# Video-Object-Detection/TSCD

Hardware: NVIDIA B200
Metric: clip-frames/sec of TSCD aggregation stage (higher is better)
Workload: dtype f16

## Files before the change

tscd_b200/aggregate.py:

```python
from typing import Dict, Optional

import torch

import os

SINGLE_PASS_MAX_LOGIT = float(os.environ.get("TSCD_ATTN_MAX_LOGIT", "25.0"))

from . import ops

FUSED_QKV = True


class MCAWeights:

    def __init__(self, sd: Dict[str, torch.Tensor], prefix: str, dtype=torch.float16, device="cuda"):
        def w(name):
            return sd[prefix + name].detach().to(device=device, dtype=dtype).contiguous()

        def b(name):
            return sd[prefix + name].detach().to(device=device, dtype=torch.float32).contiguous()

        self.qkv_cls = torch.cat([w("mca.q_cls_local.weight"), w("mca.kv_cls.weight")], 0).contiguous()
        self.qkv_reg = torch.cat([w("mca.q_reg_local.weight"), w("mca.kv_reg.weight")], 0).contiguous()
        self.lin_w, self.lin_b = w("mca.linear.weight"), b("mca.linear.bias")
        self.has_reg = (prefix + "mca.linear_reg.weight") in sd
        if self.has_reg:
            self.linreg_w, self.linreg_b = w("mca.linear_reg.weight"), b("mca.linear_reg.bias")
            self.obj_w, self.obj_b = w("linear_obj.weight"), b("linear_obj.bias")
        self.out_w, self.out_b = w("linear.weight"), b("linear.bias")


def make_layout(sel_count: torch.Tensor, B: int, F: int, L: int, row_cap: int, loc_cap: int, nk_pitch: int,
                dtype=torch.float16, row_off: Optional[torch.Tensor] = None) -> ops.AttnLayoutT:
    if row_off is None:
        cnt = sel_count.view(B, F).to(torch.int32)
        row_off = torch.zeros(B * F + 1, dtype=torch.int32, device=sel_count.device)
        row_off[1:] = torch.cumsum(cnt.reshape(-1), 0)
    lrow_off = torch.empty(B * L + 1, dtype=torch.int32, device=sel_count.device)
    assert sel_count.dtype == torch.int32 and sel_count.is_contiguous()
    ops.call("tscd_local_offsets", ops.L.LocalOffsetsArgs, B=B, F=F, L=L, sel_count=sel_count, lrow_off=lrow_off)
    return ops.AttnLayoutT(B, F, L, row_off, lrow_off, row_cap, loc_cap, nk_pitch, dtype)


def mca_forward(lay: ops.AttnLayoutT, w: MCAWeights, bank_cls, bank_reg, bank_score, n_rows_dev, n_loc_dev,
                need_reg=True, sim_thresh=0.75, conf_sim_thresh=0.99, debug=None, cls_out=(True, True), obj_out=(True, True),
                tag="mca"):
    dev, dt = bank_cls.device, lay.dtype
    tmp_c = torch.empty(lay.loc_cap, 512, dtype=dt, device=dev)
    tmp_r = torch.empty(lay.loc_cap, 512, dtype=dt, device=dev)
    qkv_c = qkv_r = None
    if FUSED_QKV:
        bufs = ops.qkv_project_fused(lay, bank_cls, bank_reg, w.qkv_cls, w.qkv_reg, bank_score, n_rows_dev,
                                     xori_cls=tmp_c[:, 256:], xori_reg=tmp_r[:, 256:], tag=tag)
    else:
        qkv_c, _ = ops.linear(bank_cls, w.qkv_cls, m_dev=n_rows_dev)
        qkv_r, _ = ops.linear(bank_reg, w.qkv_reg, m_dev=n_rows_dev)
        bufs = ops.attn_prep(lay, qkv_c, qkv_r, bank_score, xori_cls=tmp_c[:, 256:], xori_reg=tmp_r[:, 256:])
    stats = torch.empty(lay.loc_cap, 16, dtype=torch.float32, device=dev)
    ops.attn_pv(lay, bufs, tmp_c[:, :256], tmp_r[:, :256], stats, need_reg=need_reg, tag=tag, max_logit=SINGLE_PASS_MAX_LOGIT)
    cat_c = torch.empty(lay.loc_cap, 768, dtype=dt, device=dev)
    ops.linear(tmp_c, w.lin_w, w.lin_b, m_dev=n_loc_dev, out16=cat_c[:, 256:], want16=False, tag=tag + ".mca_linear")
    w_keep = torch.empty(lay.loc_cap, lay.nk_pitch, dtype=dt, device=dev) if need_reg else None
    ops.attn_round2(lay, bufs, bufs["vt_cls"], stats, cat_c[:, :256], use_obj_mask=False, sim_thresh=sim_thresh,
                    conf_sim_thresh=conf_sim_thresh, w_out=w_keep, tag=tag + ".cls")
    trans_cls16, trans_cls32 = ops.linear(cat_c, w.out_w, w.out_b, m_dev=n_loc_dev, want16=cls_out[0], want32=cls_out[1],
                                          tag=tag + ".linear")
    trans_obj16 = trans_obj32 = None
    cat_r = None
    if need_reg:
        cat_r = torch.empty(lay.loc_cap, 768, dtype=dt, device=dev)
        ops.linear(tmp_r, w.linreg_w, w.linreg_b, m_dev=n_loc_dev, out16=cat_r[:, 256:], want16=False, tag=tag + ".mca_linear_reg")
        ops.attn_round2(lay, bufs, bufs["vt_reg"], stats, cat_r[:, :256], use_obj_mask=True, sim_thresh=sim_thresh,
                        conf_sim_thresh=conf_sim_thresh, w_in=w_keep, tag=tag + ".obj")
        trans_obj16, trans_obj32 = ops.linear(cat_r, w.obj_w, w.obj_b, m_dev=n_loc_dev, want16=obj_out[0], want32=obj_out[1],
                                              tag=tag + ".linear_obj")
    if debug is not None:
        debug.update(qkv_c=qkv_c, qkv_r=qkv_r, bufs=bufs, tmp_c=tmp_c, tmp_r=tmp_r, stats=stats, cat_c=cat_c, cat_r=cat_r)
    return (trans_cls16, trans_cls32), (trans_obj16, trans_obj32)


class MSAWeights:

    def __init__(self, sd: Dict[str, torch.Tensor], prefix: str, dtype=torch.float16, device="cuda"):
        w = lambda n: sd[prefix + n].detach().to(device=device, dtype=dtype).contiguous()
        b = lambda n: sd[prefix + n].detach().to(device=device, dtype=torch.float32).contiguous()
        self.qkv_cls, self.qkv_reg = w("msa.qkv_cls.weight"), w("msa.qkv_reg.weight")
        self.l1_w, self.l1_b = w("linear1.weight"), b("linear1.bias")
        self.l2_w, self.l2_b = w("linear2.weight"), b("linear2.bias")


def msa_forward(lay: ops.AttnLayoutT, w: MSAWeights, bank_cls, bank_reg, bank_score, n_rows_dev,
                sim_thresh=0.75, conf_sim_thresh=0.99):
    assert lay.self_attn and lay.L == lay.F
    dev, dt, cap = bank_cls.device, lay.dtype, lay.row_cap
    qkv_c, _ = ops.linear(bank_cls, w.qkv_cls, m_dev=n_rows_dev, tag="msa.qkv_cls")
    qkv_r, _ = ops.linear(bank_reg, w.qkv_reg, m_dev=n_rows_dev, tag="msa.qkv_reg")
    tmp_c = torch.empty(cap, 512, dtype=dt, device=dev)
    tmp_r = torch.empty(cap, 512, dtype=dt, device=dev)
    bufs = ops.attn_prep(lay, qkv_c, qkv_r, bank_score, xori_cls=tmp_c[:, 256:], xori_reg=tmp_r[:, 256:])
    stats = torch.empty(cap, 16, dtype=torch.float32, device=dev)
    ops.attn_pv(lay, bufs, tmp_c[:, :256], tmp_r[:, :256], stats, need_reg=False, tag="msa", max_logit=SINGLE_PASS_MAX_LOGIT)
    cat = torch.empty(cap, 1024, dtype=dt, device=dev)
    ops.linear(tmp_c, w.l1_w, w.l1_b, m_dev=n_rows_dev, out16=cat[:, 512:], want16=False, tag="msa.linear1")
    tct = torch.empty(lay.B * 512, lay.nk_pitch, dtype=dt, device=dev)
    ops.call("tscd_transpose_clip", ops.L.TransposeArgs, lay=lay.to_c(), width=512, x=cat[:, 512:], ld_x=cat.stride(0), xt=tct)
    for half in range(2):
# ... 6 lines not shown
```

tscd_b200/csrc/attn.cu:

```cuda
#include <cuda.h>

#include "common.cuh"
#include "tc.cuh"

namespace tscd {

int make_tmap_kmajor(CUtensorMap* m, const void* ptr, int is_bf16, int64_t rows, int64_t K, int64_t ld, int box_rows);

constexpr int kAttnThreads = 160;
constexpr float kLog2e = 1.4426950408889634f;

template <typename T>
__device__ __forceinline__ float2 ld2(const T* p);
template <> __device__ __forceinline__ float2 ld2<__half>(const __half* p) { return __half22float2(*reinterpret_cast<const __half2*>(p)); }
template <> __device__ __forceinline__ float2 ld2<__nv_bfloat16>(const __nv_bfloat16* p) {
    return __bfloat1622float2(*reinterpret_cast<const __nv_bfloat162*>(p));
}
template <typename T>
__device__ __forceinline__ void st2(T* p, float a, float b);
template <> __device__ __forceinline__ void st2<__half>(__half* p, float a, float b) { *reinterpret_cast<__half2*>(p) = __floats2half2_rn(a, b); }
template <> __device__ __forceinline__ void st2<__nv_bfloat16>(__nv_bfloat16* p, float a, float b) {
    *reinterpret_cast<__nv_bfloat162*>(p) = __floats2bfloat162_rn(a, b);
}

// ... 966 lines not shown
        tmem_dealloc<512>(tmem);
    }
}

static bool layout_ok(const tscd_attn_layout& l) {
    return l.B > 0 && l.F > 0 && l.L > 0 && l.L <= l.F && l.row_cap > 0 && l.nk_pitch > 0 && (l.nk_pitch % 128) == 0 &&
           l.row_off && l.lrow_off && (l.dtype == TSCD_F16 || l.dtype == TSCD_BF16);
}

}

extern "C" int tscd_attn_prep(const tscd_attn_prep_args* a, void* stream) {
    using namespace tscd;
    if (!a || !layout_ok(a->lay)) return TSCD_ERR_INVALID_ARG;
    cudaStream_t st = reinterpret_cast<cudaStream_t>(stream);
    dim3 grid(a->lay.nk_pitch / 64, a->lay.B);
    const size_t smem = 2 * 64 * kPrepRowPitch * 2;
    if (a->lay.dtype == TSCD_F16) {
        if (cudaFuncSetAttribute(attn_prep_kernel<__half>, cudaFuncAttributeMaxDynamicSharedMemorySize, (int)smem) != cudaSuccess) return TSCD_ERR_CUDA;
        attn_prep_kernel<__half><<<grid, kPrepThreads, smem, st>>>(*a);
    } else {
        if (cudaFuncSetAttribute(attn_prep_kernel<__nv_bfloat16>, cudaFuncAttributeMaxDynamicSharedMemorySize, (int)smem) != cudaSuccess) return TSCD_ERR_CUDA;
        attn_prep_kernel<__nv_bfloat16><<<grid, kPrepThreads, smem, st>>>(*a);
    }
    TSCD_CUDA_CHECK_LAUNCH();
    return TSCD_OK;
}

extern "C" int tscd_transpose_clip(const tscd_transpose_args* a, void* stream) {
    using namespace tscd;
    if (!a || !layout_ok(a->lay) || a->width <= 0 || (a->width % 64) != 0) return TSCD_ERR_INVALID_ARG;
    dim3 grid(a->lay.nk_pitch / 64, a->width / 64, a->lay.B);
    cudaStream_t st = reinterpret_cast<cudaStream_t>(stream);
    if (a->lay.dtype == TSCD_F16) transpose_clip_kernel<__half><<<grid, 256, 0, st>>>(*a);
    else transpose_clip_kernel<__nv_bfloat16><<<grid, 256, 0, st>>>(*a);
    TSCD_CUDA_CHECK_LAUNCH();
    return TSCD_OK;
}

extern "C" int tscd_attn_pv(const tscd_attn_pv_args* a, void* stream) {
    using namespace tscd;
    if (!a || !layout_ok(a->lay)) return TSCD_ERR_INVALID_ARG;
    const tscd_attn_layout& l = a->lay;
    const int bf = l.dtype == TSCD_BF16;
    PvTmaps tm;
    int rc = 0;
    rc |= make_tmap_kmajor(&tm.qc, a->qn_cls, bf, l.row_cap, 256, 256, 128);
    rc |= make_tmap_kmajor(&tm.kc, a->kn_cls, bf, l.row_cap, 256, 256, 128);
    rc |= make_tmap_kmajor(&tm.qr, a->qn_reg, bf, l.row_cap, 256, 256, 128);
    rc |= make_tmap_kmajor(&tm.kr, a->kn_reg, bf, l.row_cap, 256, 256, 128);
    rc |= make_tmap_kmajor(&tm.k64c, a->kn_cls, bf, l.row_cap, 256, 256, 64);
    rc |= make_tmap_kmajor(&tm.k64r, a->kn_reg, bf, l.row_cap, 256, 256, 64);
    rc |= make_tmap_kmajor(&tm.vtc, a->vt_cls, bf, (int64_t)l.B * 256, l.nk_pitch, l.nk_pitch, 64);
    rc |= make_tmap_kmajor(&tm.vtr, a->vt_reg, bf, (int64_t)l.B * 256, l.nk_pitch, l.nk_pitch, 64);
    if (rc) return TSCD_ERR_CUDA;
    const size_t smem = 65536 + kPvStages * 32768 + 65536 + sizeof(PvBars);
    dim3 grid((l.nk_pitch + 127) / 128, l.B);
    cudaStream_t st = reinterpret_cast<cudaStream_t>(stream);
    if (bf) {
        if (cudaFuncSetAttribute(attn_pv_kernel<true>, cudaFuncAttributeMaxDynamicSharedMemorySize, (int)smem) != cudaSuccess) return TSCD_ERR_CUDA;
        attn_pv_kernel<true><<<grid, kPvThreads, smem, st>>>(tm, *a);
    } else {
        if (cudaFuncSetAttribute(attn_pv_kernel<false>, cudaFuncAttributeMaxDynamicSharedMemorySize, (int)smem) != cudaSuccess) return TSCD_ERR_CUDA;
        attn_pv_kernel<false><<<grid, kPvThreads, smem, st>>>(tm, *a);
    }
    TSCD_CUDA_CHECK_LAUNCH();
    return TSCD_OK;
}

extern "C" int tscd_attn_round2(const tscd_attn_round2_args* a, void* stream) {
    using namespace tscd;
    if (!a || !layout_ok(a->lay)) return TSCD_ERR_INVALID_ARG;
    if (a->w_in && !a->use_obj_mask) return TSCD_ERR_INVALID_ARG;
    const tscd_attn_layout& l = a->lay;
    const int bf = l.dtype == TSCD_BF16;
    R2Tmaps tm;
    int rc = 0;
    rc |= make_tmap_kmajor(&tm.q128c, a->qn_cls, bf, l.row_cap, 256, 256, 128);
    rc |= make_tmap_kmajor(&tm.q128r, a->qn_reg, bf, l.row_cap, 256, 256, 128);
    rc |= make_tmap_kmajor(&tm.k64c, a->kn_cls, bf, l.row_cap, 256, 256, 64);
    rc |= make_tmap_kmajor(&tm.k64r, a->kn_reg, bf, l.row_cap, 256, 256, 64);
    rc |= make_tmap_kmajor(&tm.vn128c, a->vn_cls, bf, l.row_cap, 256, 256, 128);
    rc |= make_tmap_kmajor(&tm.vn128r, a->vn_reg, bf, l.row_cap, 256, 256, 128);
    rc |= make_tmap_kmajor(&tm.vn64c, a->vn_cls, bf, l.row_cap, 256, 256, 64);
    rc |= make_tmap_kmajor(&tm.vn64r, a->vn_reg, bf, l.row_cap, 256, 256, 64);
    rc |= make_tmap_kmajor(&tm.vt, a->vt, bf, (int64_t)l.B * 256, l.nk_pitch, l.nk_pitch, 64);
    if (rc) return TSCD_ERR_CUDA;
    const size_t smem = kR2SmemBytes + sizeof(R2Bars);
    dim3 grid((l.nk_pitch + 127) / 128, l.B);
    cudaStream_t st = reinterpret_cast<cudaStream_t>(stream);
    if (bf) {
        if (cudaFuncSetAttribute(attn_round2_kernel<true>, cudaFuncAttributeMaxDynamicSharedMemorySize, (int)smem) != cudaSuccess) return TSCD_ERR_CUDA;
        attn_round2_kernel<true><<<grid, kR2Threads, smem, st>>>(tm, *a);
    } else {
        if (cudaFuncSetAttribute(attn_round2_kernel<false>, cudaFuncAttributeMaxDynamicSharedMemorySize, (int)smem) != cudaSuccess) return TSCD_ERR_CUDA;
        attn_round2_kernel<false><<<grid, kR2Threads, smem, st>>>(tm, *a);
    }
    TSCD_CUDA_CHECK_LAUNCH();
    return TSCD_OK;
}

#ifdef TSCD_R2_PROF
extern "C" int tscd_debug_r2_waits(unsigned long long* out, int reset) {
    if (reset) {
        unsigned long long z[64] = {};
        return cudaMemcpyToSymbol(tscd::g_r2_wait, z, sizeof(z)) == cudaSuccess && cudaMemcpyToSymbol(tscd::g_pv_wait, z, sizeof(z)) == cudaSuccess ? 0 : -1;
    }
// ... 16 lines not shown
```

tscd_b200/csrc/gemm.cu:

```cuda
#include <cuda.h>

#include "common.cuh"
#include "tc.cuh"

namespace tscd {

constexpr int kGemmBM = 128;
constexpr int kGemmBK = 64;
constexpr int kGemmStages = 3;
constexpr int kGemmThreads = 320;
constexpr int kGemmThreadsFused = 576;
__host__ __device__ constexpr int gemm_epi_warps(int epi) { return epi ? 16 : 8; }

struct GemmParams {
    int M, N, K;
    const int* m_dev;
    const float* bias;
    void* out16;
    float* out32;
    int ld16, ld32;
    int is_bf16;
    const int32_t* row_meta;
    const int32_t* row_off;
    const int32_t* lrow_off;
    int F, L, self_attn, nk_pitch;
    const float* key_score;
    float scale;
    void *qn, *kn, *vn, *vt, *xori;
    int ld_xori;
};

#ifdef TSCD_R2_PROF
__device__ unsigned long long g_gemm_wait[8];
template <int EPI>
__device__ __forceinline__ void gemm_wait_prof(uint64_t* bar, uint32_t parity, int tag, int slot) {
    const long long t0 = clock64();
    tc::mbar_wait(bar, parity, tag);
    if (EPI == 1 && blockIdx.x == 0 && (threadIdx.x & 31) == 0 && threadIdx.x < 96) atomicAdd(&g_gemm_wait[slot], (unsigned long long)(clock64() - t0));
}
#define GEMM_WAIT(bar, parity, tag, slot) gemm_wait_prof<EPI>(bar, parity, tag, slot)
#else
#define GEMM_WAIT(bar, parity, tag, slot) mbar_wait(bar, parity, tag)
#endif

constexpr int kAccStages = 2;

template <int BN, bool BF16, int EPI = 0>
__global__ void __launch_bounds__(EPI ? kGemmThreadsFused : kGemmThreads) gemm_tn_kernel(const __grid_constant__ CUtensorMap tmap_a,
                                                                const __grid_constant__ CUtensorMap tmap_w,
                                                                const GemmParams p) {
    using namespace tc;
    constexpr int STAGES = BN == 256 ? 4 : 3;
    int M = p.M;
    if (p.m_dev) M = min(M, __ldg(p.m_dev));
    const int tiles_n = (p.N + BN - 1) / BN;
    const int tiles_m = (M + kGemmBM - 1) / kGemmBM;
    const int num_tiles = tiles_m * tiles_n;
    if ((int)blockIdx.x >= num_tiles) return;
#ifdef TSCD_R2_PROF
    const long long tk0 = clock64();
#endif

    extern __shared__ __align__(1024) unsigned char smem_raw[];
    unsigned char* smem = smem_raw;
    constexpr int kABytes = kGemmBM * kGemmBK * 2;
    constexpr int kWBytes = BN * kGemmBK * 2;
    unsigned char* sA = smem;
    unsigned char* sW = smem + STAGES * kABytes;
    unsigned char* sStage = sW + STAGES * kWBytes;
    uint64_t* full_bar = reinterpret_cast<uint64_t*>(sStage + gemm_epi_warps(EPI) * 2048);
    uint64_t* empty_bar = full_bar + STAGES;
    uint64_t* tmem_full_bar = empty_bar + STAGES;
    uint64_t* tmem_empty_bar = tmem_full_bar + kAccStages;
    uint32_t& tmem_base_smem = *reinterpret_cast<uint32_t*>(tmem_empty_bar + kAccStages);
    if ((smem_u32(smem) & 1023u) != 0) __trap();

    const int warp = threadIdx.x >> 5;
    const int lane = threadIdx.x & 31;
    const int num_kb = (p.K + kGemmBK - 1) / kGemmBK;
    const bool w_resident = num_kb == STAGES;
    auto tile_origin = [&](int t, int& m0, int& n0) {
        if (w_resident) { m0 = (t % tiles_m) * kGemmBM; n0 = (t / tiles_m) * BN; }
        else { m0 = (t / tiles_n) * kGemmBM; n0 = (t % tiles_n) * BN; }
    };

    if (warp == 0 && lane == 0) {
        tma_prefetch_desc(&tmap_a);
        tma_prefetch_desc(&tmap_w);
        for (int s = 0; s < STAGES; ++s) { mbar_init(&full_bar[s], 1); mbar_init(&empty_bar[s], 1); }
        for (int s = 0; s < kAccStages; ++s) { mbar_init(&tmem_full_bar[s], 1); mbar_init(&tmem_empty_bar[s], gemm_epi_warps(EPI)); }
        fence_barrier_init();
    }
    if (warp == 1) tmem_alloc<kAccStages * BN>(&tmem_base_smem);
    tc_fence_before();
    __syncthreads();
    tc_fence_after();
    const uint32_t tmem_base = tmem_base_smem;

    if (warp == 0) {
        if (lane == 0) {
            uint32_t it = 0;
            int n_prev = -1;
            for (int t = blockIdx.x; t < num_tiles; t += gridDim.x) {
                int m0, n0;
                tile_origin(t, m0, n0);
                const bool load_w = !(w_resident && n0 == n_prev);
                for (int kb = 0; kb < num_kb; ++kb, ++it) {
                    const int s = it % STAGES;
                    const uint32_t ph = (it / STAGES) & 1;
                    GEMM_WAIT(&empty_bar[s], ph ^ 1, 100 + s, 0);
                    mbar_expect_tx(&full_bar[s], load_w ? kABytes + kWBytes : kABytes);
                    tma_load_2d(sA + s * kABytes, &tmap_a, &full_bar[s], kb * kGemmBK, m0);
                    if (load_w) tma_load_2d(sW + s * kWBytes, &tmap_w, &full_bar[s], kb * kGemmBK, n0);
                }
                n_prev = n0;
            }
        }
    } else if (warp == 1) {
        {
            const uint32_t idesc = make_idesc_f16(BF16, kGemmBM, BN);
            uint32_t it = 0, ti = 0;
            for (int t = blockIdx.x; t < num_tiles; t += gridDim.x, ++ti) {
                const int acc = ti % kAccStages;
                const uint32_t aph = (ti / kAccStages) & 1;
                GEMM_WAIT(&tmem_empty_bar[acc], aph ^ 1, 130 + acc, 1);
                tc_fence_after();
                const uint32_t d = tmem_base + (uint32_t)(acc * BN);
                for (int kb = 0; kb < num_kb; ++kb, ++it) {
                    const int s = it % STAGES;
                    const uint32_t ph = (it / STAGES) & 1;
                    GEMM_WAIT(&full_bar[s], ph, 110 + s, 2);
                    tc_fence_after();
                    const uint64_t adesc = make_smem_desc_sw128(smem_u32(sA + s * kABytes));
                    const uint64_t bdesc = make_smem_desc_sw128(smem_u32(sW + s * kWBytes));
                    if (elect_one()) {
#pragma unroll
                        for (int k = 0; k < kGemmBK / 16; ++k) {
                            umma_f16(d, adesc + (uint64_t)(k * 2), bdesc + (uint64_t)(k * 2), idesc, (kb | k) ? 1u : 0u);
                        }
                        umma_commit(&empty_bar[s]);
                    }
                    __syncwarp();
                }
                if (elect_one()) umma_commit(&tmem_full_bar[acc]);
                __syncwarp();
            }
        }
    } else {
        const int q = warp & 3;
        const int half = (warp - 2) >> 2;
        constexpr int kChunks = BN / 64;
        unsigned char* stg = sStage + (warp - 2) * 2048;
        const bool al16 = p.out16 && (p.ld16 % 8) == 0 && (reinterpret_cast<uintptr_t>(p.out16) & 15) == 0;
        const bool al32 = p.out32 && (p.ld32 % 4) == 0 && (reinterpret_cast<uintptr_t>(p.out32) & 15) == 0;
        uint32_t ti = 0;
        for (int t = blockIdx.x; t < num_tiles; t += gridDim.x, ++ti) {
            int m0, n0;
            tile_origin(t, m0, n0);
            const int acc = ti % kAccStages;
            const uint32_t aph = (ti / kAccStages) & 1;
            const int row_base = m0 + q * 32;
            const int row = row_base + lane;
            const bool row_ok = row < M;
            int meta = -1, lb = 0;
            bool is_query = false;
            if constexpr (EPI == 1) {
                meta = row_ok ? __ldg(p.row_meta + row) : -1;
                if (meta >= 0) {
                    const int cb0 = meta >> 16;
                    const int s0 = __ldg(p.row_off + cb0 * p.F);
                    const int n_loc = (p.self_attn ? __ldg(p.row_off + (cb0 + 1) * p.F) : __ldg(p.row_off + cb0 * p.F + p.L)) - s0;
                    is_query = (meta & 0xffff) < n_loc;
                    lb = __ldg(p.lrow_off + cb0 * p.L);
                }
            }
            GEMM_WAIT(&tmem_full_bar[acc], aph, 120 + acc, 3);
            tc_fence_after();
            const uint32_t tsrc = tmem_base + ((uint32_t)(q * 32) << 16) + (uint32_t)(acc * BN + half * (BN / 2));
            if constexpr (EPI == 1) {
                static_assert(BN == 256 || EPI == 0, "the fused epilogue works on 256-column tiles");
                const int kind = n0 >> 8;
                const bool valid = meta >= 0;
                const int cb = valid ? (meta >> 16) : 0, kr = meta & 0xffff;
                auto pk2h = [](float a, float b) -> uint32_t {
                    if (BF16) { __nv_bfloat162 h = __floats2bfloat162_rn(a, b); return *reinterpret_cast<uint32_t*>(&h); }
                    __half2 h = __floats2half2_rn(a, b);
                    return *reinterpret_cast<uint32_t*>(&h);
                };
                {
                    const int head = (warp - 2) >> 2;
                    const uint32_t tsrc_h = tmem_base + ((uint32_t)(q * 32) << 16) + (uint32_t)(acc * BN + head * 64);
                    uint32_t r0[32], r1[32];
                    tmem_ld_32x32(tsrc_h, r0);
                    tmem_ld_32x32(tsrc_h + 32u, r1);
                    tmem_ld_wait();
                    float ss = 0.f;
#pragma unroll
                    for (int j = 0; j < 32; ++j) {
                        ss = fmaf(__uint_as_float(r0[j]), __uint_as_float(r0[j]), ss);
                        ss = fmaf(__uint_as_float(r1[j]), __uint_as_float(r1[j]), ss);
                    }
                    auto staged_store = [&](const uint32_t (&w16)[16], uint16_t* base, int64_t dest, int ld, int col) {
                        __syncwarp();
#pragma unroll
                        for (int j = 0; j < 4; ++j)
                            *reinterpret_cast<uint4*>(stg + lane * 64 + ((j ^ ((lane >> 1) & 3)) << 4)) =
                                make_uint4(w16[4 * j], w16[4 * j + 1], w16[4 * j + 2], w16[4 * j + 3]);
                        __syncwarp();
#pragma unroll
                        for (int k = 0; k < 4; ++k) {
                            const int rr = 8 * k + (lane >> 2), ch = lane & 3;
                            const uint4 val = *reinterpret_cast<const uint4*>(stg + rr * 64 + ((ch ^ ((rr >> 1) & 3)) << 4));
                            const long long d = __shfl_sync(0xffffffffu, (long long)dest, rr);
                            if (d >= 0) *reinterpret_cast<uint4*>(base + d * ld + col + ch * 8) = val;
                        }
                    };
                    float sc = valid ? 1.f / sqrtf(ss) : 0.f;
                    if (kind == 1 && valid) sc *= p.key_score ? p.scale * __ldg(p.key_score + row) : p.scale;
                    uint16_t* nbase = reinterpret_cast<uint16_t*>(kind == 0 ? p.qn : (kind == 1 ? p.kn : p.vn));
                    const int64_t ndest = (valid && (kind != 0 || is_query)) ? (int64_t)row : -1;
                    uint32_t w16[16];
#pragma unroll
                    for (int j = 0; j < 16; ++j) w16[j] = pk2h(__uint_as_float(r0[2 * j]) * sc, __uint_as_float(r0[2 * j + 1]) * sc);
                    staged_store(w16, nbase, ndest, 256, head * 64);
#pragma unroll
                    for (int j = 0; j < 16; ++j) w16[j] = pk2h(__uint_as_float(r1[2 * j]) * sc, __uint_as_float(r1[2 * j + 1]) * sc);
                    staged_store(w16, nbase, ndest, 256, head * 64 + 32);
                    if (kind == 2) {
                        if (p.xori) {
                            const int64_t xdest = (valid && is_query) ? (int64_t)(lb + kr) : -1;
#pragma unroll
                            for (int j = 0; j < 16; ++j) w16[j] = pk2h(__uint_as_float(r0[2 * j]), __uint_as_float(r0[2 * j + 1]));
                            staged_store(w16, reinterpret_cast<uint16_t*>(p.xori), xdest, p.ld_xori, head * 64);
#pragma unroll
                            for (int j = 0; j < 16; ++j) w16[j] = pk2h(__uint_as_float(r1[2 * j]), __uint_as_float(r1[2 * j + 1]));
                            staged_store(w16, reinterpret_cast<uint16_t*>(p.xori), xdest, p.ld_xori, head * 64 + 32);
                        }
                        if (valid) {
                            uint16_t* vt = reinterpret_cast<uint16_t*>(p.vt) + ((int64_t)cb * 256 + head * 64) * p.nk_pitch + kr;
#pragma unroll
                            for (int j = 0; j < 32; ++j) {
                                vt[(int64_t)j * p.nk_pitch] = (uint16_t)(pk2h(__uint_as_float(r0[j]), 0.f) & 0xffffu);
                                vt[(int64_t)(32 + j) * p.nk_pitch] = (uint16_t)(pk2h(__uint_as_float(r1[j]), 0.f) & 0xffffu);
                            }
                        }
                    }
                    __syncwarp();
                }
                tc_fence_before();
                __syncwarp();
                if (lane == 0) mbar_arrive(&tmem_empty_bar[acc]);
                continue;
            }
            uint32_t rbuf[2][32];
            tmem_ld_32x32(tsrc, rbuf[0]);
            tmem_ld_wait();
#pragma unroll
            for (int c = 0; c < kChunks; ++c) {
                if (c + 1 < kChunks) tmem_ld_32x32(tsrc + (uint32_t)((c + 1) * 32), rbuf[(c + 1) & 1]);
                const uint32_t* r = rbuf[c & 1];
                const int col0 = n0 + half * (BN / 2) + c * 32;
                if (col0 < p.N) {
                    float v[32];
                    if (p.bias) {
#pragma unroll
                        for (int j = 0; j < 32; ++j) v[j] = __uint_as_float(r[j]) + ((col0 + j < p.N) ? __ldg(p.bias + col0 + j) : 0.f);
                    } else {
#pragma unroll
                        for (int j = 0; j < 32; ++j) v[j] = __uint_as_float(r[j]);
                    }
                    const bool full = (col0 + 32 <= p.N);
                    if (p.out16) {
                        uint32_t pk[16];
#pragma unroll
                        for (int j = 0; j < 16; ++j) {
                            if (BF16) {
                                __nv_bfloat162 h = __floats2bfloat162_rn(v[2 * j], v[2 * j + 1]);
                                pk[j] = *reinterpret_cast<uint32_t*>(&h);
                            } else {
                                __half2 h = __floats2half2_rn(v[2 * j], v[2 * j + 1]);
                                pk[j] = *reinterpret_cast<uint32_t*>(&h);
                            }
                        }
                        uint16_t* obase = reinterpret_cast<uint16_t*>(p.out16);
                        __syncwarp();
#pragma unroll
                        for (int j = 0; j < 4; ++j)
                            *reinterpret_cast<uint4*>(stg + lane * 64 + ((j ^ ((lane >> 1) & 3)) << 4)) =
                                make_uint4(pk[4 * j], pk[4 * j + 1], pk[4 * j + 2], pk[4 * j + 3]);
                        __syncwarp();
                        if (full && al16) {
// ... 38 lines not shown
                    }
                }
                if (c + 1 < kChunks) tmem_ld_wait();
            }
            tc_fence_before();
            __syncwarp();
            if (lane == 0) mbar_arrive(&tmem_empty_bar[acc]);
        }
    }
#ifdef TSCD_R2_PROF
    if (EPI == 1 && blockIdx.x == 0 && (threadIdx.x & 31) == 0 && threadIdx.x < 96) atomicAdd(&g_gemm_wait[4 + warp], (unsigned long long)(clock64() - tk0));
#endif
    tc_fence_before();
    __syncthreads();
    if (warp == 1) {
        tc_fence_after();
        tmem_dealloc<kAccStages * BN>(tmem_base);
    }
}

typedef CUresult (*PFN_encodeTiled)(CUtensorMap*, CUtensorMapDataType, cuuint32_t, void*, const cuuint64_t*,
                                    const cuuint64_t*, const cuuint32_t*, const cuuint32_t*, CUtensorMapInterleave,
                                    CUtensorMapSwizzle, CUtensorMapL2promotion, CUtensorMapFloatOOBfill);

static PFN_encodeTiled get_encode() {
    static PFN_encodeTiled fn = nullptr;
    if (!fn) {
        void* p = nullptr;
        cudaDriverEntryPointQueryResult q;
        if (cudaGetDriverEntryPoint("cuTensorMapEncodeTiled", &p, cudaEnableDefault, &q) != cudaSuccess) return nullptr;
        if (q != cudaDriverEntryPointSuccess) return nullptr;
        fn = reinterpret_cast<PFN_encodeTiled>(p);
    }
    return fn;
}

int make_tmap_kmajor(CUtensorMap* m, const void* ptr, int is_bf16, int64_t rows, int64_t K, int64_t ld, int box_rows) {
    PFN_encodeTiled enc = get_encode();
    if (!enc) return TSCD_ERR_CUDA;
    if ((ld * 2) % 16 != 0 || (reinterpret_cast<uintptr_t>(ptr) & 15) != 0) return TSCD_ERR_INVALID_ARG;
    cuuint64_t dims[2] = {(cuuint64_t)K, (cuuint64_t)rows};
    cuuint64_t strides[1] = {(cuuint64_t)(ld * 2)};
    cuuint32_t box[2] = {(cuuint32_t)kGemmBK, (cuuint32_t)box_rows};
    cuuint32_t estr[2] = {1, 1};
    CUresult r = enc(m, is_bf16 ? CU_TENSOR_MAP_DATA_TYPE_BFLOAT16 : CU_TENSOR_MAP_DATA_TYPE_FLOAT16, 2,
                     const_cast<void*>(ptr), dims, strides, box, estr, CU_TENSOR_MAP_INTERLEAVE_NONE,
                     CU_TENSOR_MAP_SWIZZLE_128B, CU_TENSOR_MAP_L2_PROMOTION_L2_256B, CU_TENSOR_MAP_FLOAT_OOB_FILL_NONE);
    return r == CUDA_SUCCESS ? TSCD_OK : TSCD_ERR_CUDA;
}

template <int BN, bool BF16, int EPI = 0>
static int launch_gemm(const CUtensorMap& ta, const CUtensorMap& tw, const GemmParams& p, cudaStream_t st) {
    constexpr int STAGES = BN == 256 ? 4 : 3;
    constexpr size_t smem = (size_t)STAGES * (kGemmBM * kGemmBK * 2 + BN * kGemmBK * 2) + gemm_epi_warps(EPI) * 2048 + 128;
    static bool attr_set[64] = {};
    static int num_sms_dev[64] = {};
    int dev = 0;
    if (cudaGetDevice(&dev) != cudaSuccess || dev < 0 || dev >= 64) return TSCD_ERR_CUDA;
    if (!attr_set[dev]) {
        if (cudaFuncSetAttribute(gemm_tn_kernel<BN, BF16, EPI>, cudaFuncAttributeMaxDynamicSharedMemorySize, (int)smem) != cudaSuccess)
            return TSCD_ERR_CUDA;
        if (cudaDeviceGetAttribute(&num_sms_dev[dev], cudaDevAttrMultiProcessorCount, dev) != cudaSuccess) return TSCD_ERR_CUDA;
        attr_set[dev] = true;
    }
    const int num_sms = num_sms_dev[dev];
    const int tiles = ((p.N + BN - 1) / BN) * ((p.M + kGemmBM - 1) / kGemmBM);
    const int ctas_per_sm = BN == 256 ? 1 : 2;
    const int grid = tiles < ctas_per_sm * num_sms ? tiles : ctas_per_sm * num_sms;
    gemm_tn_kernel<BN, BF16, EPI><<<grid, EPI ? kGemmThreadsFused : kGemmThreads, smem, st>>>(ta, tw, p);
    return cudaGetLastError() == cudaSuccess ? TSCD_OK : TSCD_ERR_CUDA;
}

}

extern "C" int tscd_linear(const tscd_linear_args* a, void* stream) {
    using namespace tscd;
    if (!a || a->M <= 0 || a->N <= 0 || a->K <= 0 || !a->x || !a->w) return TSCD_ERR_INVALID_ARG;
    if (a->dtype != TSCD_F16 && a->dtype != TSCD_BF16) return TSCD_ERR_UNSUPPORTED;
    if (!a->out16 && !a->out32) return TSCD_ERR_INVALID_ARG;
    const int is_bf16 = a->dtype == TSCD_BF16;
    const int BN = a->N <= 64 ? 64 : ((a->N % 256) == 0 && a->K >= 256 ? 256 : 128);
    CUtensorMap ta, tw;
    int rc = make_tmap_kmajor(&ta, a->x, is_bf16, a->M, a->K, a->ldx, kGemmBM);
    if (rc != TSCD_OK) return rc;
    rc = make_tmap_kmajor(&tw, a->w, is_bf16, a->N, a->K, a->ldw, BN);
    if (rc != TSCD_OK) return rc;
    GemmParams p = {};
    p.M = a->M; p.N = a->N; p.K = a->K;
    p.m_dev = a->m_dev; p.bias = a->bias;
    p.out16 = a->out16; p.out32 = a->out32;
    p.ld16 = a->ld16; p.ld32 = a->ld32;
    p.is_bf16 = is_bf16;
    cudaStream_t st = reinterpret_cast<cudaStream_t>(stream);
    if (is_bf16) return BN == 64 ? launch_gemm<64, true>(ta, tw, p, st) : (BN == 128 ? launch_gemm<128, true>(ta, tw, p, st) : launch_gemm<256, true>(ta, tw, p, st));
    return BN == 64 ? launch_gemm<64, false>(ta, tw, p, st) : (BN == 128 ? launch_gemm<128, false>(ta, tw, p, st) : launch_gemm<256, false>(ta, tw, p, st));
}

extern "C" int tscd_qkv_project(const tscd_qkv_project_args* a, void* stream) {
    using namespace tscd;
    if (!a || a->rows <= 0 || !a->x || !a->w || !a->row_meta || !a->qn || !a->kn || !a->vn || !a->vt) return TSCD_ERR_INVALID_ARG;
    const tscd_attn_layout& l = a->lay;
    if (l.dtype != TSCD_F16 && l.dtype != TSCD_BF16) return TSCD_ERR_UNSUPPORTED;
    if (l.B <= 0 || l.F <= 0 || l.L <= 0 || l.L > l.F || !l.row_off || !l.lrow_off || (l.nk_pitch % 128) != 0 || l.nk_pitch > 65536) return TSCD_ERR_INVALID_ARG;
    const int is_bf16 = l.dtype == TSCD_BF16;
    CUtensorMap ta, tw;
    int rc = make_tmap_kmajor(&ta, a->x, is_bf16, a->rows, 256, a->ldx, kGemmBM);
    if (rc != TSCD_OK) return rc;
    rc = make_tmap_kmajor(&tw, a->w, is_bf16, 768, 256, 256, 256);
    if (rc != TSCD_OK) return rc;
    GemmParams p = {};
    p.M = a->rows; p.N = 768; p.K = 256;
    p.m_dev = a->m_dev;
    p.is_bf16 = is_bf16;
    p.row_meta = a->row_meta; p.row_off = l.row_off; p.lrow_off = l.lrow_off;
    p.F = l.F; p.L = l.L; p.self_attn = l.self_attn; p.nk_pitch = l.nk_pitch;
    p.key_score = a->key_score; p.scale = a->scale;
    p.qn = a->qn; p.kn = a->kn; p.vn = a->vn; p.vt = a->vt; p.xori = a->xori; p.ld_xori = a->ld_xori;
    cudaStream_t st = reinterpret_cast<cudaStream_t>(stream);
    return is_bf16 ? launch_gemm<256, true, 1>(ta, tw, p, st) : launch_gemm<256, false, 1>(ta, tw, p, st);
}

#ifdef TSCD_R2_PROF
extern "C" int tscd_debug_gemm_waits(unsigned long long* out, int reset) {
    if (reset) {
        unsigned long long z[8] = {};
        return cudaMemcpyToSymbol(tscd::g_gemm_wait, z, sizeof(z)) == cudaSuccess ? 0 : -1;
    }
    return cudaMemcpyFromSymbol(out, tscd::g_gemm_wait, sizeof(unsigned long long) * 8) == cudaSuccess ? 0 : -1;
}
#endif
```

tscd_b200/ops.py:

```python
import ctypes as C
from dataclasses import dataclass
from typing import List, Optional, Sequence

import torch

from . import _lib as L

_DT = {torch.float32: L.TSCD_F32, torch.float16: L.TSCD_F16, torch.bfloat16: L.TSCD_BF16}


def _stream():
    return C.c_void_p(torch.cuda.current_stream().cuda_stream)


def _p(t: Optional[torch.Tensor]):
    return C.c_void_p(0 if t is None else t.data_ptr())


@dataclass
class AnchorSpec:
    hw: Sequence[Sequence[int]]
    strides: Sequence[int] = (8, 16, 32)

    @property
# ... 345 lines not shown
    if bias is not None:
        assert bias.dtype == torch.float32 and bias.is_contiguous()
    if L.profile is not None:
        L.profile.setdefault("linear", []).append((M, N, K, m_dev, tag, out16 is not None, out32 is not None))
    with L.timed("tscd_linear", tag):
        L.check(L.lib().tscd_linear(C.byref(a), _stream()), "tscd_linear")
    return out16, out32


@dataclass
class AttnLayoutT:
    B: int
    F: int
    L: int
    row_off: torch.Tensor
    lrow_off: torch.Tensor
    row_cap: int
    loc_cap: int
    nk_pitch: int
    dtype: torch.dtype
    self_attn: bool = False

    def to_c(self) -> L.AttnLayout:
        a = L.AttnLayout()
        a.B, a.F, a.L, a.self_attn, a.dtype = self.B, self.F, self.L, int(self.self_attn), _DT[self.dtype]
        a.row_cap, a.nk_pitch = self.row_cap, self.nk_pitch
        a.row_off, a.lrow_off = _p(self.row_off), _p(self.lrow_off)
        return a


def attn_prep(lay: AttnLayoutT, qkv_cls, qkv_reg, key_score, xori_cls=None, xori_reg=None, scale=25.0, bufs=None):
    dev, dt = qkv_cls.device, lay.dtype
    if bufs is None:
        bufs = {}
        for n in ("qn_cls", "kn_cls", "vn_cls", "qn_reg", "kn_reg", "vn_reg"):
            bufs[n] = torch.empty(lay.row_cap, 256, dtype=dt, device=dev)
        for n in ("vt_cls", "vt_reg"):
            bufs[n] = torch.empty(lay.B * 256, lay.nk_pitch, dtype=dt, device=dev)
        bufs["row_frame"] = torch.empty(lay.row_cap, dtype=torch.int32, device=dev)
    a = L.AttnPrepArgs()
    a.lay, a.scale = lay.to_c(), scale
    assert qkv_cls.stride(1) == 1 and qkv_cls.stride(0) == qkv_reg.stride(0)
    a.qkv_cls, a.qkv_reg, a.ld_qkv, a.key_score = _p(qkv_cls), _p(qkv_reg), qkv_cls.stride(0), _p(key_score)
    for n in ("qn_cls", "kn_cls", "vn_cls", "qn_reg", "kn_reg", "vn_reg", "vt_cls", "vt_reg", "row_frame"):
        setattr(a, n, _p(bufs[n]))
    a.xori_cls, a.xori_reg = _p(xori_cls), _p(xori_reg)
    a.ld_xori = 0 if xori_cls is None else xori_cls.stride(0)
    with L.timed("tscd_attn_prep"):
        L.check(L.lib().tscd_attn_prep(C.byref(a), _stream()), "tscd_attn_prep")
    return bufs


def qkv_project_fused(lay: AttnLayoutT, bank_cls, bank_reg, w_cls, w_reg, key_score, n_rows_dev, xori_cls=None, xori_reg=None,
                      scale=25.0, tag=None):
    dev, dt = bank_cls.device, lay.dtype
    bufs = {}
    for n in ("qn_cls", "kn_cls", "vn_cls", "qn_reg", "kn_reg", "vn_reg"):
        bufs[n] = torch.empty(lay.row_cap, 256, dtype=dt, device=dev)
    for n in ("vt_cls", "vt_reg"):
        bufs[n] = torch.empty(lay.B * 256, lay.nk_pitch, dtype=dt, device=dev)
    bufs["row_frame"] = torch.empty(lay.row_cap, dtype=torch.int32, device=dev)
    bufs["row_meta"] = torch.empty(lay.row_cap, dtype=torch.int32, device=dev)
    call("tscd_attn_rowmeta", L.AttnRowmetaArgs, lay=lay.to_c(), row_frame=bufs["row_frame"], row_meta=bufs["row_meta"],
         vt_cls=bufs["vt_cls"], vt_reg=bufs["vt_reg"])
    for br, bank, w, ks, xo in (("cls", bank_cls, w_cls, key_score, xori_cls), ("reg", bank_reg, w_reg, None, xori_reg)):
        assert bank.shape[0] >= lay.row_cap and bank.stride(1) == 1 and w.shape == (768, 256) and w.is_contiguous()
        call("tscd_qkv_project", L.QkvProjectArgs, tag=None if tag is None else f"{tag}.{br}", lay=lay.to_c(), rows=lay.row_cap, m_dev=n_rows_dev, x=bank, ldx=bank.stride(0),
             w=w, row_meta=bufs["row_meta"], key_score=ks, scale=scale, qn=bufs["qn_" + br], kn=bufs["kn_" + br],
             vn=bufs["vn_" + br], vt=bufs["vt_" + br], xori=xo, ld_xori=0 if xo is None else xo.stride(0))
    return bufs


def attn_pv(lay: AttnLayoutT, bufs, x_cls, x_reg, stats, need_reg=True, tag=None, max_logit: float = 0.0):
    a = L.AttnPvArgs()
    a.max_logit = max_logit
    a.lay = lay.to_c()
    for n in ("qn_cls", "kn_cls", "qn_reg", "kn_reg", "vt_cls", "vt_reg", "row_frame"):
        setattr(a, n, _p(bufs[n]))
    a.need_reg = int(need_reg)
    a.x_cls, a.x_reg, a.ld_x, a.stats = _p(x_cls), _p(x_reg), x_cls.stride(0), _p(stats)
    with L.timed("tscd_attn_pv", tag):
        L.check(L.lib().tscd_attn_pv(C.byref(a), _stream()), "tscd_attn_pv")


def attn_round2(lay: AttnLayoutT, bufs, vt, stats, out, use_obj_mask, sim_thresh=0.75, conf_sim_thresh=0.99, w_out=None, w_in=None,
                tag=None):
    a = L.AttnRound2Args()
    a.lay = lay.to_c()
    for n in ("qn_cls", "kn_cls", "qn_reg", "kn_reg", "vn_cls", "vn_reg", "row_frame"):
        setattr(a, n, _p(bufs[n]))
    a.vt, a.stats, a.use_obj_mask = _p(vt), _p(stats), int(use_obj_mask)
    a.sim_thresh, a.conf_sim_thresh = sim_thresh, conf_sim_thresh
    a.out, a.ld_out = _p(out), out.stride(0)
    a.w_out, a.w_in = _p(w_out), _p(w_in)
    for t in (w_out, w_in):
        assert t is None or (t.dtype == lay.dtype and t.stride(0) == lay.nk_pitch and t.stride(1) == 1)
    with L.timed("tscd_attn_round2", tag):
        L.check(L.lib().tscd_attn_round2(C.byref(a), _stream()), "tscd_attn_round2")


def call(name: str, struct_cls, tag=None, **kw):
    a = struct_cls()
    for k, v in kw.items():
        if isinstance(v, C.Structure):
            pass
        elif isinstance(v, torch.Tensor) or v is None:
            v = _p(v)
        elif isinstance(v, torch.dtype):
            v = _DT[v]
        setattr(a, k, v)
    missing = {f[0] for f in struct_cls._fields_} - set(kw)
    assert not missing, f"{name}: missing {missing}"
    with L.timed(name, tag):
        L.check(getattr(L.lib(), name)(C.byref(a), _stream()), name)


def frame_scatter(store, frame_slots: torch.Tensor, sel: dict, status: torch.Tensor, slot_error: Optional[torch.Tensor] = None):
    a = L.FrameScatterArgs()
    a.store = store.to_c()
    a.num_frames = frame_slots.numel()
    a.frame_slots, a.status, a.slot_error = _p(frame_slots), _p(status), _p(slot_error)
    for k in ("sel_count", "row_off", "sel_idx", "sel_rows", "bank_cls", "bank_reg", "bank_edge", "bank_score"):
        setattr(a, k, _p(sel[k]))
    with L.timed("tscd_frame_scatter"):
        L.check(L.lib().tscd_frame_scatter(C.byref(a), _stream()), "tscd_frame_scatter")


def clip_assemble(store, clip_slots: torch.Tensor, B: int, F: int, Lf: int, row_cap: int, status: torch.Tensor,
                  out: Optional[dict] = None, want_idx: bool = True) -> dict:
    dev = clip_slots.device
    nf, kmax, W = B * F, store.kmax, 7 + store.num_classes
# ... 14 lines not shown
```

Measured before the change: 1.525 million.

## Skip Q tiles without queries and drop unused reg outputs in fused QKV GEMM

The fused QKV projection GEMM now schedules its work in groups of three CTAs per M-tile strip. Each member handles the Q, K or V column block in a rotating pattern. A per-CTA flag table in shared memory marks M tiles that contain no query rows, so their Q-column tiles are skipped. When the regression branch is not needed, the reg VT transpose buffer and xori output are no longer allocated or written, and attn_pv falls back to the cls VT map. This removes wasted GEMM and store work, at the cost of a fixed grid size that may leave SMs idle or unbalance the load.

```diff
diff --git a/tscd_b200/aggregate.py b/tscd_b200/aggregate.py
--- a/tscd_b200/aggregate.py
+++ b/tscd_b200/aggregate.py
@@ -51,7 +51,8 @@
     qkv_c = qkv_r = None
     if FUSED_QKV:
         bufs = ops.qkv_project_fused(lay, bank_cls, bank_reg, w.qkv_cls, w.qkv_reg, bank_score, n_rows_dev,
-                                     xori_cls=tmp_c[:, 256:], xori_reg=tmp_r[:, 256:], tag=tag)
+                                     xori_cls=tmp_c[:, 256:], xori_reg=tmp_r[:, 256:] if need_reg else None, tag=tag,
+                                     need_reg=need_reg)
     else:
         qkv_c, _ = ops.linear(bank_cls, w.qkv_cls, m_dev=n_rows_dev)
         qkv_r, _ = ops.linear(bank_reg, w.qkv_reg, m_dev=n_rows_dev)
diff --git a/tscd_b200/csrc/attn.cu b/tscd_b200/csrc/attn.cu
--- a/tscd_b200/csrc/attn.cu
+++ b/tscd_b200/csrc/attn.cu
@@ -1042,7 +1042,8 @@
     rc |= make_tmap_kmajor(&tm.k64c, a->kn_cls, bf, l.row_cap, 256, 256, 64);
     rc |= make_tmap_kmajor(&tm.k64r, a->kn_reg, bf, l.row_cap, 256, 256, 64);
     rc |= make_tmap_kmajor(&tm.vtc, a->vt_cls, bf, (int64_t)l.B * 256, l.nk_pitch, l.nk_pitch, 64);
-    rc |= make_tmap_kmajor(&tm.vtr, a->vt_reg, bf, (int64_t)l.B * 256, l.nk_pitch, l.nk_pitch, 64);
+    if (a->need_reg && !a->vt_reg) return TSCD_ERR_INVALID_ARG;
+    rc |= make_tmap_kmajor(&tm.vtr, a->need_reg ? a->vt_reg : a->vt_cls, bf, (int64_t)l.B * 256, l.nk_pitch, l.nk_pitch, 64);
     if (rc) return TSCD_ERR_CUDA;
     const size_t smem = 65536 + kPvStages * 32768 + 65536 + sizeof(PvBars);
     dim3 grid((l.nk_pitch + 127) / 128, l.B);
diff --git a/tscd_b200/csrc/gemm.cu b/tscd_b200/csrc/gemm.cu
--- a/tscd_b200/csrc/gemm.cu
+++ b/tscd_b200/csrc/gemm.cu
@@ -23,7 +23,7 @@
     const int32_t* row_meta;
     const int32_t* row_off;
     const int32_t* lrow_off;
-    int F, L, self_attn, nk_pitch;
+    int B, F, L, self_attn, nk_pitch;
     const float* key_score;
     float scale;
     void *qn, *kn, *vn, *vt, *xori;
@@ -44,6 +44,9 @@
 #endif
 
 constexpr int kAccStages = 2;
+
+constexpr int kQkvGroup = 3;
+constexpr int kQFlagCap = 2048;
 
 template <int BN, bool BF16, int EPI = 0>
 __global__ void __launch_bounds__(EPI ? kGemmThreadsFused : kGemmThreads) gemm_tn_kernel(const __grid_constant__ CUtensorMap tmap_a,
@@ -56,7 +59,10 @@
     const int tiles_n = (p.N + BN - 1) / BN;
     const int tiles_m = (M + kGemmBM - 1) / kGemmBM;
     const int num_tiles = tiles_m * tiles_n;
-    if ((int)blockIdx.x >= num_tiles) return;
+    const int groups = EPI ? (int)gridDim.x / kQkvGroup : 0;
+    const int grp = EPI ? (int)blockIdx.x / kQkvGroup : 0, member = EPI ? (int)blockIdx.x % kQkvGroup : 0;
+    const int rounds = EPI ? (tiles_m + groups - 1) / groups : 0;
+    if (EPI ? grp >= tiles_m : (int)blockIdx.x >= num_tiles) return;
 #ifdef TSCD_R2_PROF
     const long long tk0 = clock64();
 #endif
@@ -79,10 +85,28 @@
     const int lane = threadIdx.x & 31;
     const int num_kb = (p.K + kGemmBK - 1) / kGemmBK;
     const bool w_resident = num_kb == STAGES;
-    auto tile_origin = [&](int t, int& m0, int& n0) {
-        if (w_resident) { m0 = (t % tiles_m) * kGemmBM; n0 = (t / tiles_m) * BN; }
-        else { m0 = (t / tiles_n) * kGemmBM; n0 = (t % tiles_n) * BN; }
+    unsigned char* qflag = reinterpret_cast<unsigned char*>(full_bar) + 128;
+    auto next_tile = [&](int& cur, int& m0, int& n0) -> bool {
+        if constexpr (EPI == 1) {
+            for (;; ++cur) {
+                const int mt = grp + groups * cur;
+                if (mt >= tiles_m) return false;
+                const int kind = (member + kQkvGroup * cur / rounds) % kQkvGroup;
+                if (kind == 0 && cur < kQFlagCap && !qflag[cur]) continue;
+                m0 = mt * kGemmBM;
+                n0 = kind * BN;
+                ++cur;
+                return true;
+            }
+        } else {
+            if (cur >= num_tiles) return false;
+            if (w_resident) { m0 = (cur % tiles_m) * kGemmBM; n0 = (cur / tiles_m) * BN; }
+            else { m0 = (cur / tiles_n) * kGemmBM; n0 = (cur % tiles_n) * BN; }
+            cur += gridDim.x;
+            return true;
+        }
     };
+    const int cur0 = EPI ? 0 : (int)blockIdx.x;
 
     if (warp == 0 && lane == 0) {
         tma_prefetch_desc(&tmap_a);
@@ -92,6 +116,28 @@
         fence_barrier_init();
     }
     if (warp == 1) tmem_alloc<kAccStages * BN>(&tmem_base_smem);
+    if constexpr (EPI == 1) {
+        if (warp >= 2) {
+            for (int r = threadIdx.x - 64; r < min(rounds, kQFlagCap); r += blockDim.x - 64) {
+                const int mt = grp + groups * r;
+                bool hq = true;
+                if (mt < tiles_m && (member + kQkvGroup * r / rounds) % kQkvGroup == 0) {
+                    const int m_end = min(M, (mt + 1) * kGemmBM);
+                    int row = mt * kGemmBM;
+                    const int meta = __ldg(p.row_meta + row);
+                    if (meta >= 0) {
+                        hq = false;
+                        for (int cb = meta >> 16; row < m_end && cb < p.B; ++cb) {
+                            const int qend = __ldg(p.row_off + (p.self_attn ? (cb + 1) * p.F : cb * p.F + p.L));
+                            if (row < qend) { hq = true; break; }
+                            row = __ldg(p.row_off + (cb + 1) * p.F);
+                        }
+                    }
+                }
+                qflag[r] = hq;
+            }
+        }
+    }
     tc_fence_before();
     __syncthreads();
     tc_fence_after();
@@ -101,9 +147,8 @@
         if (lane == 0) {
             uint32_t it = 0;
             int n_prev = -1;
-            for (int t = blockIdx.x; t < num_tiles; t += gridDim.x) {
-                int m0, n0;
-                tile_origin(t, m0, n0);
+            int cur = cur0, m0, n0;
+            while (next_tile(cur, m0, n0)) {
                 const bool load_w = !(w_resident && n0 == n_prev);
                 for (int kb = 0; kb < num_kb; ++kb, ++it) {
                     const int s = it % STAGES;
@@ -120,7 +165,8 @@
         {
             const uint32_t idesc = make_idesc_f16(BF16, kGemmBM, BN);
             uint32_t it = 0, ti = 0;
-            for (int t = blockIdx.x; t < num_tiles; t += gridDim.x, ++ti) {
+            int cur = cur0, m0, n0;
+            for (; next_tile(cur, m0, n0); ++ti) {
                 const int acc = ti % kAccStages;
                 const uint32_t aph = (ti / kAccStages) & 1;
                 GEMM_WAIT(&tmem_empty_bar[acc], aph ^ 1, 130 + acc, 1);
@@ -154,9 +200,8 @@
         const bool al16 = p.out16 && (p.ld16 % 8) == 0 && (reinterpret_cast<uintptr_t>(p.out16) & 15) == 0;
         const bool al32 = p.out32 && (p.ld32 % 4) == 0 && (reinterpret_cast<uintptr_t>(p.out32) & 15) == 0;
         uint32_t ti = 0;
-        for (int t = blockIdx.x; t < num_tiles; t += gridDim.x, ++ti) {
-            int m0, n0;
-            tile_origin(t, m0, n0);
+        int cur = cur0, m0, n0;
+        for (; next_tile(cur, m0, n0); ++ti) {
             const int acc = ti % kAccStages;
             const uint32_t aph = (ti / kAccStages) & 1;
             const int row_base = m0 + q * 32;
@@ -236,7 +281,7 @@
                             for (int j = 0; j < 16; ++j) w16[j] = pk2h(__uint_as_float(r1[2 * j]), __uint_as_float(r1[2 * j + 1]));
                             staged_store(w16, reinterpret_cast<uint16_t*>(p.xori), xdest, p.ld_xori, head * 64 + 32);
                         }
-                        if (valid) {
+                        if (valid && p.vt) {
                             uint16_t* vt = reinterpret_cast<uint16_t*>(p.vt) + ((int64_t)cb * 256 + head * 64) * p.nk_pitch + kr;
 #pragma unroll
                             for (int j = 0; j < 32; ++j) {
@@ -381,7 +426,8 @@
 template <int BN, bool BF16, int EPI = 0>
 static int launch_gemm(const CUtensorMap& ta, const CUtensorMap& tw, const GemmParams& p, cudaStream_t st) {
     constexpr int STAGES = BN == 256 ? 4 : 3;
-    constexpr size_t smem = (size_t)STAGES * (kGemmBM * kGemmBK * 2 + BN * kGemmBK * 2) + gemm_epi_warps(EPI) * 2048 + 128;
+    constexpr size_t smem = (size_t)STAGES * (kGemmBM * kGemmBK * 2 + BN * kGemmBK * 2) + gemm_epi_warps(EPI) * 2048 + 128 +
+                            (EPI ? kQFlagCap : 0);
     static bool attr_set[64] = {};
     static int num_sms_dev[64] = {};
     int dev = 0;
@@ -395,7 +441,11 @@
     const int num_sms = num_sms_dev[dev];
     const int tiles = ((p.N + BN - 1) / BN) * ((p.M + kGemmBM - 1) / kGemmBM);
     const int ctas_per_sm = BN == 256 ? 1 : 2;
-    const int grid = tiles < ctas_per_sm * num_sms ? tiles : ctas_per_sm * num_sms;
+    int grid = tiles < ctas_per_sm * num_sms ? tiles : ctas_per_sm * num_sms;
+    if (EPI) {
+        const int tiles_m = (p.M + kGemmBM - 1) / kGemmBM;
+        grid = kQkvGroup * min(tiles_m, num_sms / kQkvGroup);
+    }
     gemm_tn_kernel<BN, BF16, EPI><<<grid, EPI ? kGemmThreadsFused : kGemmThreads, smem, st>>>(ta, tw, p);
     return cudaGetLastError() == cudaSuccess ? TSCD_OK : TSCD_ERR_CUDA;
 }
@@ -427,7 +477,7 @@
 
 extern "C" int tscd_qkv_project(const tscd_qkv_project_args* a, void* stream) {
     using namespace tscd;
-    if (!a || a->rows <= 0 || !a->x || !a->w || !a->row_meta || !a->qn || !a->kn || !a->vn || !a->vt) return TSCD_ERR_INVALID_ARG;
+    if (!a || a->rows <= 0 || !a->x || !a->w || !a->row_meta || !a->qn || !a->kn || !a->vn) return TSCD_ERR_INVALID_ARG;
     const tscd_attn_layout& l = a->lay;
     if (l.dtype != TSCD_F16 && l.dtype != TSCD_BF16) return TSCD_ERR_UNSUPPORTED;
     if (l.B <= 0 || l.F <= 0 || l.L <= 0 || l.L > l.F || !l.row_off || !l.lrow_off || (l.nk_pitch % 128) != 0 || l.nk_pitch > 65536) return TSCD_ERR_INVALID_ARG;
@@ -442,7 +492,7 @@
     p.m_dev = a->m_dev;
     p.is_bf16 = is_bf16;
     p.row_meta = a->row_meta; p.row_off = l.row_off; p.lrow_off = l.lrow_off;
-    p.F = l.F; p.L = l.L; p.self_attn = l.self_attn; p.nk_pitch = l.nk_pitch;
+    p.B = l.B; p.F = l.F; p.L = l.L; p.self_attn = l.self_attn; p.nk_pitch = l.nk_pitch;
     p.key_score = a->key_score; p.scale = a->scale;
     p.qn = a->qn; p.kn = a->kn; p.vn = a->vn; p.vt = a->vt; p.xori = a->xori; p.ld_xori = a->ld_xori;
     cudaStream_t st = reinterpret_cast<cudaStream_t>(stream);
diff --git a/tscd_b200/ops.py b/tscd_b200/ops.py
--- a/tscd_b200/ops.py
+++ b/tscd_b200/ops.py
@@ -421,22 +421,23 @@
 
 
 def qkv_project_fused(lay: AttnLayoutT, bank_cls, bank_reg, w_cls, w_reg, key_score, n_rows_dev, xori_cls=None, xori_reg=None,
-                      scale=25.0, tag=None):
+                      scale=25.0, tag=None, bufs=None, need_reg=True):
     dev, dt = bank_cls.device, lay.dtype
-    bufs = {}
-    for n in ("qn_cls", "kn_cls", "vn_cls", "qn_reg", "kn_reg", "vn_reg"):
-        bufs[n] = torch.empty(lay.row_cap, 256, dtype=dt, device=dev)
-    for n in ("vt_cls", "vt_reg"):
-        bufs[n] = torch.empty(lay.B * 256, lay.nk_pitch, dtype=dt, device=dev)
-    bufs["row_frame"] = torch.empty(lay.row_cap, dtype=torch.int32, device=dev)
-    bufs["row_meta"] = torch.empty(lay.row_cap, dtype=torch.int32, device=dev)
+    if bufs is None:
+        bufs = {}
+        for n in ("qn_cls", "kn_cls", "vn_cls", "qn_reg", "kn_reg", "vn_reg"):
+            bufs[n] = torch.empty(lay.row_cap, 256, dtype=dt, device=dev)
+        for n in ("vt_cls", "vt_reg")[:2 if need_reg else 1]:
+            bufs[n] = torch.empty(lay.B * 256, lay.nk_pitch, dtype=dt, device=dev)
+        bufs["row_frame"] = torch.empty(lay.row_cap, dtype=torch.int32, device=dev)
+        bufs["row_meta"] = torch.empty(lay.row_cap, dtype=torch.int32, device=dev)
     call("tscd_attn_rowmeta", L.AttnRowmetaArgs, lay=lay.to_c(), row_frame=bufs["row_frame"], row_meta=bufs["row_meta"],
-         vt_cls=bufs["vt_cls"], vt_reg=bufs["vt_reg"])
+         vt_cls=bufs["vt_cls"], vt_reg=bufs.get("vt_reg"))
     for br, bank, w, ks, xo in (("cls", bank_cls, w_cls, key_score, xori_cls), ("reg", bank_reg, w_reg, None, xori_reg)):
         assert bank.shape[0] >= lay.row_cap and bank.stride(1) == 1 and w.shape == (768, 256) and w.is_contiguous()
         call("tscd_qkv_project", L.QkvProjectArgs, tag=None if tag is None else f"{tag}.{br}", lay=lay.to_c(), rows=lay.row_cap, m_dev=n_rows_dev, x=bank, ldx=bank.stride(0),
              w=w, row_meta=bufs["row_meta"], key_score=ks, scale=scale, qn=bufs["qn_" + br], kn=bufs["kn_" + br],
-             vn=bufs["vn_" + br], vt=bufs["vt_" + br], xori=xo, ld_xori=0 if xo is None else xo.stride(0))
+             vn=bufs["vn_" + br], vt=bufs.get("vt_" + br), xori=xo, ld_xori=0 if xo is None else xo.stride(0))
     return bufs
 
 
@@ -445,7 +446,7 @@
     a.max_logit = max_logit
     a.lay = lay.to_c()
     for n in ("qn_cls", "kn_cls", "qn_reg", "kn_reg", "vt_cls", "vt_reg", "row_frame"):
-        setattr(a, n, _p(bufs[n]))
+        setattr(a, n, _p(bufs.get(n)))
     a.need_reg = int(need_reg)
     a.x_cls, a.x_reg, a.ld_x, a.stats = _p(x_cls), _p(x_reg), x_cls.stride(0), _p(stats)
     with L.timed("tscd_attn_pv", tag):
```

New measurement: 1.578 million, median of 6. +3.5%, better.
